# ZhuoyangLiu2005/MLA

Hardware: AMD Instinct MI355X
Metric: training samples/sec + step-time, MLA-Llama2-7B bf16 (higher is better)
Workload: dtype bf16; 1 GPU; BASELINE.json configs[1]: MLA-Llama2-7B SFT, use_pointcloud+use_contrastive, 672x672(+mask) image + 1024 points + 32 text tokens, per-GPU batch 8 x 4 diffusion repeats = 32 x 548 tokens; model=mla-llama2-7b, global_batch=8, seq_len=548, parallelism=single-gpu, activation_save_level=1, optimizer=fused AdamW + grad clip inside the timed region

## Files before the change

include/mla_hip.h:

```cpp
#ifndef MLA_HIP_H
#define MLA_HIP_H

#include <stddef.h>
#include <stdint.h>

#ifdef __cplusplus
extern "C" {
#endif

typedef struct ihipStream_t* mla_stream_t;

const char* mla_last_error(void);
int mla_query(int what);
const char* mla_gemm_source_id(void);
int mla_selftest(const void* src_1k, int* out_tr_256, void* out_glds_1k, mla_stream_t stream);
int mla_calib_mfma(const void* operands, float* out, int blocks, int iters, double* flops_per_launch, mla_stream_t stream);
int mla_dispatch_probe(int* out, int blocks, int hold_us, mla_stream_t stream);

int mla_gemm_bf16(const void* A, const void* B, void* C, const void* R, const void* bias, int M, int N, int K, int lda, int ldb,
                  int ldc, int ldr, int a_mode, int b_mode, int out_fp32, int accumulate, float alpha, int force_generic,
                  mla_stream_t stream);
int mla_gemm_bf16_ws(const void* A, const void* B, void* C, const void* R, const void* bias, int M, int N, int K, int lda, int ldb,
                     int ldc, int ldr, int a_mode, int b_mode, int out_fp32, int accumulate, float alpha, int force_generic,
                     float* workspace, size_t workspace_bytes, mla_stream_t stream);
// ... 32 lines not shown
int mla_colsum_blocks(int rows);
int mla_colsum_bf16(const void* dy, float* out, int accumulate, int rows, int N, int ld, float* workspace, size_t workspace_bytes,
                    mla_stream_t stream);
int mla_layernorm_fwd(const void* x, const void* w, const void* b, void* y, int rows, int H, float eps, mla_stream_t stream);

int mla_rope_inplace(void* buf, const float* cos_t, const float* sin_t, long long tokens, int S, int nheads, int D, int ld,
                     int q_off, int k_off, int backward, mla_stream_t stream);

int mla_swiglu_fwd(const void* gu, void* act, long long rows, int I, mla_stream_t stream);
int mla_swiglu_bwd(const void* dact, const void* gu, void* dgu, void* act_out, long long rows, int I, mla_stream_t stream);
int mla_act_fwd(const void* x, void* y, long long n, int kind, mla_stream_t stream);
int mla_act_bwd(const void* dy, const void* x, void* dx, long long n, int kind, mla_stream_t stream);

int mla_cast_f32_to_bf16(const float* x, void* y, long long n, mla_stream_t stream);
int mla_cast_bf16_to_f32(const void* x, float* y, long long n, mla_stream_t stream);
int mla_add_bf16(const void* a, const void* b, void* y, long long n, mla_stream_t stream);
int mla_gather_rows_bf16(const void* src, const long long* idx, void* out, long long rows, int H, int scatter, mla_stream_t stream);

int mla_transpose_bf16(const void* src, void* dst, long long R, int C, long long ld, long long ldt, mla_stream_t stream);
int mla_rmsnorm_apply_t(const void* x, const void* w, const float* rstd, void* dst, long long rows, int H, long long ldt,
                        mla_stream_t stream);
int mla_swiglu_fwd_t(const void* gu, void* dst, long long rows, int I, long long ldt, mla_stream_t stream);
int mla_swiglu_fwd_dual(const void* gu, void* act, void* actT, long long rows, int I, long long ldt, mla_stream_t stream);
int mla_swiglu_bwd_t(const void* dact, const void* gu, void* dgu, void* dguT, long long rows, int I, long long ldt, mla_stream_t stream);

int mla_embedding_fwd(const long long* ids, const void* table, void* out, long long tokens, int H, int vocab, mla_stream_t stream);
int mla_embedding_bwd(const long long* ids, const void* dy, float* grad, float* workspace, long long tokens, int H, int vocab,
                      mla_stream_t stream);

int mla_adamw_step(float* p, const float* g, float* m, float* v, void* p16, long long n, float lr, float beta1, float beta2,
                   float eps, float weight_decay, int step, const float* grad_scale, mla_stream_t stream);
int mla_adamw_step_groups(float* p, const float* g, float* m, float* v, void* p16, long long n, long long n_decay, float lr, float beta1,
                          float beta2, float eps, float weight_decay, int step, const float* grad_scale, mla_stream_t stream);
int mla_sumsq_f32(const float* x, long long n, float* out, int accumulate, float* workspace, size_t workspace_bytes,
                  mla_stream_t stream);
int mla_sum_partials(const float* partial, int n, float* out, int accumulate, mla_stream_t stream);
int mla_clip_coef(const float* sumsq, float max_norm, float* coef, float* norm_out, mla_stream_t stream);

int mla_q_sample(const float* x0, const float* noise, const long long* t, const float* sqrt_ac, const float* sqrt_1mac, float* out,
                 int batch, int per, int nsteps, mla_stream_t stream);

int mla_attn_fwd(const void* q, const void* k, const void* v, void* o, float* lse, const int* seqlens, int B, int S, int H,
                 int head_dim, long long ld_qkv, long long ld_o, float scale, mla_stream_t stream);
int mla_attn_fwd_g(const void* q, const void* k, const void* v, void* o, float* lse, const int* seqlens, int B, int S, int H,
                   int head_dim, long long ld_qkv, long long ld_o, float scale, int grp_start, int grp_len, const int* grp_starts,
                   mla_stream_t stream);
int mla_attn_bwd_g(const void* q, const void* k, const void* v, const void* o, const void* dout, const float* lse, const int* seqlens,
                   void* dq, void* dk, void* dv, float* delta, int B, int S, int H, int head_dim, long long ld_qkv, long long ld_o,
                   float scale, const float* rope_cos, const float* rope_sin, void* dqT, void* dkT, void* dvT, void* oT,
                   long long ldt, int* head_sync, long long head_sync_ints, int grp_start, int grp_len, const int* grp_starts,
                   int rope_per_sample, mla_stream_t stream);
long long mla_attn_bwd_sync_ints(int B, int H);
int mla_attn_bwd(const void* q, const void* k, const void* v, const void* o, const void* dout, const float* lse, const int* seqlens,
                 void* dq, void* dk, void* dv, float* delta, int B, int S, int H, int head_dim, long long ld_qkv, long long ld_o,
                 float scale, const float* rope_cos, const float* rope_sin, int* head_sync, long long head_sync_ints,
                 mla_stream_t stream);
int mla_attn_bwd_t(const void* q, const void* k, const void* v, const void* o, const void* dout, const float* lse, const int* seqlens,
                   void* dq, void* dk, void* dv, float* delta, int B, int S, int H, int head_dim, long long ld_qkv, long long ld_o,
                   float scale, const float* rope_cos, const float* rope_sin, void* dqT, void* dkT, void* dvT, void* oT,
                   long long ldt, int* head_sync, long long head_sync_ints, mla_stream_t stream);
long long mla_attn_bwd_ws_bytes(int B, int S, int H);
int mla_attn_bwd_ws(const void* q, const void* k, const void* v, const void* o, const void* dout, const float* lse, const int* seqlens,
                    void* dq, void* dk, void* dv, float* delta, int B, int S, int H, int head_dim, long long ld_qkv, long long ld_o,
                    float scale, const float* rope_cos, const float* rope_sin, void* dqT, void* dkT, void* dvT, void* oT, long long ldt,
                    void* ws, long long ws_bytes, mla_stream_t stream);

// ... 93 lines not shown
```

mla_amd/csrc/elementwise.hip:

```cpp
#include "common.h"
#include <math.h>

namespace {


constexpr int NORM_MAXC = 4;

__global__ __launch_bounds__(256) void rmsnorm_fwd_kernel(const bf16_t* __restrict__ x, const bf16_t* __restrict__ w,
                                                          bf16_t* __restrict__ y, float* __restrict__ rstd_out,
                                                          int rows, int H, float eps) {
  __shared__ float scratch[16];
  const int row = blockIdx.x;
  const int nchunk = H >> 3;
  const bf16_t* xr = x + (size_t)row * H;
  float xv[NORM_MAXC][8];
  float ss = 0.f;
#pragma unroll
  for (int c = 0; c < NORM_MAXC; ++c) {
    const int ch = threadIdx.x + c * 256;
    if (ch < nchunk) {
      const u32x4_t v = *(const u32x4_t*)(xr + ch * 8);
      unpack8(v, xv[c]);
#pragma unroll
      for (int j = 0; j < 8; ++j) ss += xv[c][j] * xv[c][j];
// ... 646 lines not shown
          g4[u] = __builtin_nontemporal_load(g + i); p4[u] = __builtin_nontemporal_load(p + i);
          m4[u] = __builtin_nontemporal_load(m + i); v4[u] = __builtin_nontemporal_load(v + i);
        } else {
          g4[u] = g[i]; p4[u] = p[i]; m4[u] = m[i]; v4[u] = v[i];
        }
      }
    }
#pragma unroll
    for (int u = 0; u < UNR; ++u) {
      const long long i = i0 + u * 256;
      if (i >= hi) continue;
      const float decay = i < n4_decay ? decay_on : 1.f;
#pragma unroll
      for (int r = 0; r < 4; ++r) {
        float pp = p4[u][r], mm = m4[u][r], vv = v4[u][r];
        adamw_elem(pp, g4[u][r], mm, vv, gs, decay, beta1, beta2, step, isq, eps);
        p4[u][r] = pp; m4[u][r] = mm; v4[u][r] = vv;
      }
      if (NT) {
        __builtin_nontemporal_store(p4[u], p + i); __builtin_nontemporal_store(m4[u], m + i); __builtin_nontemporal_store(v4[u], v + i);
      } else {
        p[i] = p4[u]; m[i] = m4[u]; v[i] = v4[u];
      }
      if (p16) {
        u32x2_t o;
        o[0] = pack2bf(p4[u][0], p4[u][1]);
        o[1] = pack2bf(p4[u][2], p4[u][3]);
        if (NT) __builtin_nontemporal_store(o, p16 + i); else p16[i] = o;
      }
    }
  }
}

__global__ __launch_bounds__(256) void sumsq_partial_kernel(const float* __restrict__ x, float* __restrict__ partial, long long n) {
  __shared__ float scratch[16];
  float s0 = 0.f, s1 = 0.f;
  const long long n4 = n >> 2;
  const f32x4_t* x4 = (const f32x4_t*)x;
  for (long long i = (long long)blockIdx.x * 256 + threadIdx.x; i < n4; i += (long long)gridDim.x * 256) {
    const f32x4_t v = x4[i];
    s0 += v[0] * v[0] + v[1] * v[1];
    s1 += v[2] * v[2] + v[3] * v[3];
  }
  if (blockIdx.x == 0 && threadIdx.x < (n & 3)) { const float v = x[(n4 << 2) + threadIdx.x]; s0 += v * v; }
  const float s = block_sum(s0 + s1, scratch);
  if (threadIdx.x == 0) partial[blockIdx.x] = s;
}
__global__ __launch_bounds__(256) void sum_final_kernel(const float* __restrict__ partial, float* __restrict__ out, int P,
                                                        int accumulate) {
  __shared__ float scratch[16];
  float s = 0.f;
  int i0 = 0;
  if ((((uintptr_t)partial) & 15) == 0) {
    const f32x4_t* p4 = (const f32x4_t*)partial;
    const int n4 = P >> 2;
    f32x4_t a0 = {0.f, 0.f, 0.f, 0.f}, a1 = a0, a2 = a0, a3 = a0;
    int i = threadIdx.x;
    for (; i + 768 < n4; i += 1024) { a0 += p4[i]; a1 += p4[i + 256]; a2 += p4[i + 512]; a3 += p4[i + 768]; }
    for (; i < n4; i += 256) a0 += p4[i];
    const f32x4_t a = (a0 + a1) + (a2 + a3);
    s = (a[0] + a[1]) + (a[2] + a[3]);
    i0 = n4 << 2;
  }
  for (int i = i0 + threadIdx.x; i < P; i += 256) s += partial[i];
  s = block_sum(s, scratch);
  if (threadIdx.x == 0) out[0] = accumulate ? out[0] + s : s;
// ... 219 lines not shown
  MLA_CHECK_ARG(p && g && m && v && n >= 0 && step >= 1 && n_decay >= 0 && n_decay <= n, "mla_adamw_step: bad args");
  if (n == 0) return 0;
  const float bc1 = 1.f - powf(beta1, (float)step), bc2 = 1.f - powf(beta2, (float)step);
  const long long n4 = (AL16(p) && AL16(g) && AL16(m) && AL16(v) && (p16 == nullptr || ((uintptr_t)p16 & 7) == 0) && (n_decay & 3) == 0) ? n / 4 : 0;
  if (n4) {
    static const int variant = getenv("MLA_ADAMW_VARIANT") ? atoi(getenv("MLA_ADAMW_VARIANT")) : 0;
    const dim3 grid(grid_for(n4, adamw_grid_cap()));
#define ADAMW_LAUNCH(U, N) hipLaunchKernelGGL((adamw_vec4_kernel<U, N>), grid, dim3(256), 0, stream, (f32x4_t*)p, (const f32x4_t*)g, (f32x4_t*)m, \
                       (f32x4_t*)v, (u32x2_t*)p16, n4, lr, beta1, beta2, eps, weight_decay, bc1, bc2, grad_scale, n_decay / 4)
    if (variant == 1) ADAMW_LAUNCH(2, true);
    else if (variant == 9) ADAMW_LAUNCH(1, true);
    else if (variant == 3) ADAMW_LAUNCH(1, false);
    else if (variant == 4) ADAMW_LAUNCH(2, false);
    else ADAMW_LAUNCH(4, true);
#undef ADAMW_LAUNCH
  }
  const long long done = n4 * 4;
  if (done < n)
    hipLaunchKernelGGL(adamw_kernel, dim3(grid_for(n - done, 8192)), dim3(256), 0, stream, p + done, g + done, m + done, v + done,
                       p16 ? (bf16_t*)p16 + done : (bf16_t*)nullptr, n - done, lr, beta1, beta2, eps, weight_decay, bc1, bc2, grad_scale,
                       n_decay > done ? n_decay - done : 0);
  MLA_LAUNCH_CHECK();
}
extern "C" int mla_adamw_step(float* p, const float* g, float* m, float* v, void* p16, long long n, float lr, float beta1,
                              float beta2, float eps, float weight_decay, int step, const float* grad_scale,
                              hipStream_t stream) {
  return adamw_impl(p, g, m, v, p16, n, n, lr, beta1, beta2, eps, weight_decay, step, grad_scale, stream);
}
extern "C" int mla_adamw_step_groups(float* p, const float* g, float* m, float* v, void* p16, long long n, long long n_decay, float lr,
                                     float beta1, float beta2, float eps, float weight_decay, int step, const float* grad_scale,
                                     hipStream_t stream) {
  return adamw_impl(p, g, m, v, p16, n, n_decay, lr, beta1, beta2, eps, weight_decay, step, grad_scale, stream);
}

extern "C" int mla_sumsq_f32(const float* x, long long n, float* out, int accumulate, float* workspace, size_t workspace_bytes,
                             hipStream_t stream) {
  MLA_CHECK_ARG(x && out && workspace && workspace_bytes >= 2048 * sizeof(float) && AL16(x), "mla_sumsq_f32: bad args");
  const int nb = grid_for(n / 4 + 1, 2048);
  hipLaunchKernelGGL(sumsq_partial_kernel, dim3(nb), dim3(256), 0, stream, x, workspace, n);
  hipLaunchKernelGGL(sum_final_kernel, dim3(1), dim3(256), 0, stream, workspace, out, nb, accumulate);
  MLA_LAUNCH_CHECK();
}
extern "C" int mla_sum_partials(const float* partial, int n, float* out, int accumulate, hipStream_t stream) {
  MLA_CHECK_ARG(partial && out && n >= 0, "mla_sum_partials: bad args");
  hipLaunchKernelGGL(sum_final_kernel, dim3(1), dim3(256), 0, stream, partial, out, n, accumulate);
  MLA_LAUNCH_CHECK();
}
extern "C" int mla_clip_coef(const float* sumsq, float max_norm, float* coef, float* norm_out, hipStream_t stream) {
  MLA_CHECK_ARG(sumsq && coef, "mla_clip_coef: bad args");
  hipLaunchKernelGGL(clip_coef_kernel, dim3(1), dim3(1), 0, stream, sumsq, max_norm, coef, norm_out);
  MLA_LAUNCH_CHECK();
}

extern "C" int mla_q_sample(const float* x0, const float* noise, const long long* t, const float* sqrt_ac,
                            const float* sqrt_1mac, float* out, int batch, int per, int nsteps, hipStream_t stream) {
  MLA_CHECK_ARG(x0 && noise && t && sqrt_ac && sqrt_1mac && out, "mla_q_sample: null pointer");
  hipLaunchKernelGGL(q_sample_kernel, dim3((batch * per + 255) / 256), dim3(256), 0, stream, x0, noise, t, sqrt_ac, sqrt_1mac,
                     out, batch, per, nsteps);
  MLA_LAUNCH_CHECK();
}

extern "C" int mla_gather_rows_bf16(const void* src, const long long* idx, void* out, long long rows, int H, int scatter,
                                    hipStream_t stream) {
  MLA_CHECK_ARG(src && idx && out && H % 8 == 0 && AL16(src) && AL16(out), "mla_gather_rows_bf16: bad args");
  hipLaunchKernelGGL(gather_rows_kernel, dim3(grid_for(rows * (H / 8))), dim3(256), 0, stream, (const bf16_t*)src, idx, (bf16_t*)out,
                     rows, H, scatter);
// ... 3 lines not shown
```

mla_amd/fsdp.py:

```python
from __future__ import annotations

from typing import Callable, Dict, List, Optional, Sequence, Tuple

import torch
import torch.distributed as dist
import torch.nn as nn


class HipLocalOps:

    def __init__(self):
        from . import hip
        self.hip = hip

    def cast_to_bf16(self, src32, dst16):
        self.hip.cast_f32_to_bf16(src32, dst16)

    def adamw(self, p32, g32, m, v, p16, lr, betas, eps, wd, step, grad_scale):
        self.hip.adamw_step(p32, g32, m, v, p16, lr, betas[0], betas[1], eps, wd, step, grad_scale)

    def adamw_groups(self, p32, g32, m, v, p16, n_decay, lr, betas, eps, wd, step, grad_scale):
        self.hip.adamw_step_groups(p32, g32, m, v, p16, n_decay, lr, betas[0], betas[1], eps, wd, step, grad_scale)

    def sumsq(self, x32, out1, accumulate):
        self.hip.sumsq(x32, out1, accumulate)

    def sum_partials(self, partials, n, out1, accumulate):
        self.hip.sum_partials(partials, n, out1, accumulate)

    def clip_coef(self, sumsq1, max_norm, coef1, norm1):
        self.hip.clip_coef(sumsq1, max_norm, coef1, norm1)

    def stream(self, device):
        return torch.cuda.Stream(device=device)


class _SqArena:

    def __init__(self, n: int, device):
        self.buf = torch.zeros(n, dtype=torch.float32, device=device)
        self.used = 0

    def take(self, count: int):
        if self.used + count > self.buf.numel():
            return None
        part = self.buf[self.used:self.used + count]
        self.used += count
        return part


def _round_up(n, m):
    return ((n + m - 1) // m) * m


def apply_rccl_env(environ=None) -> Dict[str, str]:
# ... 284 lines not shown
        self.world = dist.get_world_size(process_group) if dist.is_available() and dist.is_initialized() else 1
        self.rank = dist.get_rank(process_group) if self.world > 1 else 0
        self.coll = self.world > 1 or (os.environ.get("MLA_FORCE_COLLECTIVES") == "1" and dist.is_available() and dist.is_initialized())
        self.ops = ops if ops is not None else HipLocalOps()
        if inplace_reduce is None and os.environ.get("MLA_FSDP_INPLACE_RS") == "0":
            inplace_reduce = False
        self.inplace_reduce = bool(self.coll and (dist.get_backend(process_group) == "nccl" if inplace_reduce is None else inplace_reduce))
        self.sum_shards = bool(self.inplace_reduce or (self.coll and dist.get_backend(process_group) == "nccl"))
        self.grad_div = float(self.world) if self.sum_shards else 1.0
        no_decay = no_decay or default_no_decay
        self.units: List[FlatUnit] = []
        self.unit_of_module: Dict[int, FlatUnit] = {}
        found = discover_units(model, unit_policy)
        self._arenas = None
        kinds = [k for k in os.environ.get("MLA_FSDP_ARENAS", "master,exp_avg,exp_avg_sq").split(",") if k and k != "0"]
        if kinds:
            sizes = dict(flat16=0, grad32=0, master=0, exp_avg=0, exp_avg_sq=0, gshard=0)
            for name, mod, named in found:
                _, n_decay, n_train, n_total = plan_flat_layout(named, self.world, no_decay)
                w = self.world if self.coll else 1
                sizes["flat16"] += n_total
                sizes["grad32"] += n_train
                sizes["master"] += n_total // w
                sizes["exp_avg"] += n_train // self.world
                sizes["exp_avg_sq"] += n_train // self.world
                if self.coll and not self.inplace_reduce:
                    sizes["gshard"] += n_train // self.world
            self._arenas = _Arenas({k: v for k, v in sizes.items() if k in kinds}, device, slices=2 * len(found))
        for name, mod, named in found:
            self._add_unit(name, mod, named, no_decay)
        for b in model.buffers():
            b.data = b.data.to(device)
        self.step_count = 0
        self.defer_reduce = False
        self._sumsq = torch.zeros(1, dtype=torch.float32, device=device)
        self._sq_arena = _SqArena(1 << 20, device) if (not self.coll and hasattr(self.ops, "sum_partials") and
                                                       self.device.type == "cuda") else None
        for u in self.units:
            u.sq_arena = self._sq_arena
        self._coef = torch.ones(1, dtype=torch.float32, device=device)
        self._norm = torch.zeros(1, dtype=torch.float32, device=device)
        self.on_gpu = self.device.type == "cuda"
        if self.on_gpu:
            assert torch.cuda.current_device() == (self.device.index or 0), \
                f"torch.cuda.set_device({self.device}) must be called before sharding a model onto it"
        self.comm_stream = self.ops.stream(device) if self.coll else None
        self.wait_profile = None
        if self.on_gpu and self.comm_stream is not None:
            for u in self.units:
                mod = getattr(u, "module", None)
                if mod is not None:
                    mod.register_forward_pre_hook(lambda m, inp, uu=u: self.wait_unit(uu))
                    if hasattr(mod, "_gather_wait"):
                        mod._gather_wait = (lambda uu=u: self.wait_unit(uu))
                else:
                    owned = {id(p) for _, p, _ in u.params}
                    for m in model.modules():
                        if any(id(p) in owned for p in m.parameters(recurse=False)):
                            m.register_forward_pre_hook(lambda mm, inp, uu=u: self.wait_unit(uu))
        for u in self.units:
            mod = getattr(u, "module", None)
            if mod is not None and hasattr(mod, "_grad_hook") and u.trainable and self.coll:
                mod._grad_hook = (lambda uu=u: self._launch_reduce_scatter(uu))

    def _add_unit(self, name, mod, named, no_decay):
        if not named:
# ... 100 lines not shown
                        self._timed_wait("rs_event", u.rs_event)

    def grad_norm_and_clip(self, max_norm: Optional[float]):
        first = True
        small: List[torch.Tensor] = []
        for u in self.units:
            if not u.trainable:
                continue
            if u.sq_entries and not self.coll:
                for a, b in u.uncovered_ranges():
                    if b - a > (1 << 20):
                        self.ops.sumsq(u.gshard[a:b], self._sumsq, not first)
                        first = False
                    else:
                        small.append(u.gshard[a:b])
            else:
                self.ops.sumsq(u.gshard, self._sumsq, not first)
                first = False
        if small:
            self.ops.sumsq(torch.cat(small) if len(small) > 1 else small[0], self._sumsq, not first)
            first = False
        if self._sq_arena is not None and self._sq_arena.used:
            self.ops.sum_partials(self._sq_arena.buf, self._sq_arena.used, self._sumsq, not first)
            first = False
        if self.coll:
            dist.all_reduce(self._sumsq, op=dist.ReduceOp.SUM, group=self.pg)
        if self.grad_div != 1.0:
            self._sumsq.mul_(1.0 / (self.grad_div * self.grad_div))
        self.ops.clip_coef(self._sumsq, float(max_norm) if max_norm is not None else 3.0e38, self._coef, self._norm)
        if self.grad_div != 1.0:
            self._coef.mul_(1.0 / self.grad_div)
        return self._norm

    def optimizer_step(self, lr: float, betas=(0.9, 0.999), eps: float = 1e-8, weight_decay: float = 0.0):
        self.step_count += 1

        for u in self.units:
            if not u.trainable:
                continue
            ranges = u._shard_ranges()
            if hasattr(self.ops, "adamw_groups") and ranges and ranges[0][0] == 0 and \
                    all(ranges[i][1] == ranges[i + 1][0] and ranges[i][2] + (ranges[i][1] - ranges[i][0]) == ranges[i + 1][2]
                        for i in range(len(ranges) - 1)):
                n_local = ranges[-1][1]
                n_dec = sum(le - ls for ls, le, _, dec in ranges if dec)
                g0 = ranges[0][2]
                self.ops.adamw_groups(u.master_train[:n_local], u.gshard[:n_local], u.exp_avg[:n_local], u.exp_avg_sq[:n_local],
                                      u.flat16[g0:g0 + n_local], n_dec, lr, betas, eps, weight_decay, self.step_count, self._coef)
            else:
                for ls, le, g0, decayed in ranges:
                    self.ops.adamw(u.master_train[ls:le], u.gshard[ls:le], u.exp_avg[ls:le], u.exp_avg_sq[ls:le],
                                   u.flat16[g0:g0 + (le - ls)], lr, betas, eps, weight_decay if decayed else 0.0, self.step_count,
                                   self._coef)
            if self.coll:
                if self.on_gpu:
                    ev = torch.cuda.Event()
                    ev.record(torch.cuda.current_stream(self.device))
                    with torch.cuda.stream(self.comm_stream):
                        self.comm_stream.wait_event(ev)
                        self._all_gather(u)
                        u.gather_event = torch.cuda.Event()
                        u.gather_event.record(self.comm_stream)
                else:
                    self._all_gather(u)

    def iter_full_state_fp32(self, to_cpu_on_rank0: bool = False):
        if self.on_gpu:
            self.wait_all()
        for u in self.units:
            full = self._gather_master(u)
            keep = (not to_cpu_on_rank0) or self.rank == 0
            for n, p, o in u.params:
                if not keep:
                    yield n, None
                    continue
                t = full[o:o + p.numel()].view(p.shape)
                yield n, (t.cpu() if to_cpu_on_rank0 else t.clone())
            del full

    def full_state_dict_fp32(self) -> Dict[str, torch.Tensor]:
        return dict(self.iter_full_state_fp32())

    def _gather_master(self, u: FlatUnit):
        if not self.coll:
            return torch.cat([u.master_train, u.master_frozen])
        full = torch.empty(u.n_total, dtype=torch.float32, device=self.device)
        parts_t = [torch.empty(u.shard_train, dtype=torch.float32, device=self.device) for _ in range(self.world)]
        dist.all_gather(parts_t, u.master_train, group=self.pg)
        full[:u.n_train] = torch.cat(parts_t)
        nf = (u.n_total - u.n_train) // self.world
        if nf:
            parts_f = [torch.empty(nf, dtype=torch.float32, device=self.device) for _ in range(self.world)]
            dist.all_gather(parts_f, u.master_frozen, group=self.pg)
            full[u.n_train:] = torch.cat(parts_f)
        return full

    def state_bytes(self):
# ... 2 lines not shown
```

mla_amd/hip.py:

```python
from __future__ import annotations

import ctypes
import os
from ctypes import c_float, c_int, c_longlong, c_size_t, c_void_p
from typing import Optional

import torch

_LIB_PATH = os.environ.get("MLA_HIP_LIB") or os.path.join(os.path.dirname(os.path.abspath(__file__)), "libmla_hip.so")
_lib = None

ACT_GELU_ERF, ACT_GELU_TANH, ACT_RELU, ACT_SILU = 0, 1, 2, 3

SPLITK = os.environ.get("MLA_GEMM_SPLITK", "1") != "0"
SPLITK_WS_BYTES = int(os.environ.get("MLA_GEMM_SPLITK_WS_MB", "64")) << 20

GEMM_PROFILE = None

_SIGNATURES = {
    "mla_query": [c_int],
    "mla_selftest": [c_void_p, c_void_p, c_void_p, c_void_p],
    "mla_dispatch_probe": [c_void_p, c_int, c_int, c_void_p],
    "mla_calib_mfma": [c_void_p, c_void_p, c_int, c_int, c_void_p, c_void_p],
    "mla_gemv_bf16": [c_void_p, c_longlong, c_void_p, c_longlong, c_void_p, c_longlong, c_longlong, c_int, c_void_p, c_longlong, c_int, c_int,
# ... 20 lines not shown
    "mla_gemm_gateup_swiglu": [c_void_p, c_void_p, c_void_p, c_void_p, c_void_p, c_int, c_int, c_int, c_int, c_int, c_longlong,
                               c_void_p],
    "mla_gemm_dact_swiglu_bwd": [c_void_p, c_void_p, c_void_p, c_void_p, c_void_p, c_int, c_int, c_int, c_int, c_int, c_longlong,
                                 c_void_p],
    "mla_rmsnorm_fwd": [c_void_p, c_void_p, c_void_p, c_void_p, c_int, c_int, c_float, c_void_p],
    "mla_rmsnorm_prep": [c_void_p, c_void_p, c_void_p, c_void_p, c_int, c_int, c_float, c_void_p],
    "mla_gemm_res_norm": [c_void_p, c_void_p, c_void_p, c_void_p, c_void_p, c_void_p, c_void_p, c_int, c_int, c_int, c_int, c_int, c_int,
                          c_int, c_void_p, c_size_t, c_void_p],
    "mla_gemm_qkv_rope_rs": [c_void_p, c_void_p, c_void_p, c_int, c_int, c_int, c_int, c_int, c_int, c_void_p, c_void_p, c_int, c_int,
                             c_void_p, c_int, c_float, c_void_p, c_void_p],
    "mla_gemm_gateup_swiglu_rs": [c_void_p, c_void_p, c_void_p, c_void_p, c_void_p, c_int, c_int, c_int, c_int, c_int, c_longlong,
                                  c_void_p, c_int, c_float, c_void_p, c_void_p],
    "mla_rmsnorm_bwd_blocks": [c_int],
    "mla_timm_rmsnorm_fwd": [c_void_p, c_void_p, c_void_p, c_void_p, c_void_p, c_int, c_int, c_float, c_void_p],
    "mla_timm_rmsnorm_bwd": [c_void_p, c_void_p, c_void_p, c_void_p, c_void_p, c_void_p, c_void_p, c_int, c_int, c_int, c_void_p,
                             c_size_t, c_void_p],
    "mla_rmsnorm_bwd": [c_void_p, c_void_p, c_void_p, c_void_p, c_void_p, c_void_p, c_void_p, c_int, c_int, c_int, c_void_p,
                        c_size_t, c_void_p],
    "mla_colsum_blocks": [c_int],
    "mla_colsum_bf16": [c_void_p, c_void_p, c_int, c_int, c_int, c_int, c_void_p, c_size_t, c_void_p],
    "mla_layernorm_fwd": [c_void_p, c_void_p, c_void_p, c_void_p, c_int, c_int, c_float, c_void_p],
    "mla_rope_inplace": [c_void_p, c_void_p, c_void_p, c_longlong, c_int, c_int, c_int, c_int, c_int, c_int, c_int, c_void_p],
    "mla_swiglu_fwd": [c_void_p, c_void_p, c_longlong, c_int, c_void_p],
    "mla_swiglu_bwd": [c_void_p, c_void_p, c_void_p, c_void_p, c_longlong, c_int, c_void_p],
    "mla_act_fwd": [c_void_p, c_void_p, c_longlong, c_int, c_void_p],
    "mla_act_bwd": [c_void_p, c_void_p, c_void_p, c_longlong, c_int, c_void_p],
    "mla_cast_f32_to_bf16": [c_void_p, c_void_p, c_longlong, c_void_p],
    "mla_cast_bf16_to_f32": [c_void_p, c_void_p, c_longlong, c_void_p],
    "mla_add_bf16": [c_void_p, c_void_p, c_void_p, c_longlong, c_void_p],
    "mla_embedding_fwd": [c_void_p, c_void_p, c_void_p, c_longlong, c_int, c_int, c_void_p],
    "mla_embedding_bwd": [c_void_p, c_void_p, c_void_p, c_void_p, c_longlong, c_int, c_int, c_void_p],
    "mla_adamw_step_groups": [c_void_p, c_void_p, c_void_p, c_void_p, c_void_p, c_longlong, c_longlong, c_float, c_float, c_float, c_float,
                              c_float, c_int, c_void_p, c_void_p],
    "mla_adamw_step": [c_void_p, c_void_p, c_void_p, c_void_p, c_void_p, c_longlong, c_float, c_float, c_float, c_float,
                       c_float, c_int, c_void_p, c_void_p],
    "mla_sumsq_f32": [c_void_p, c_longlong, c_void_p, c_int, c_void_p, c_size_t, c_void_p],
    "mla_clip_coef": [c_void_p, c_float, c_void_p, c_void_p, c_void_p],
    "mla_q_sample": [c_void_p, c_void_p, c_void_p, c_void_p, c_void_p, c_void_p, c_int, c_int, c_int, c_void_p],
    "mla_attn_fwd": [c_void_p, c_void_p, c_void_p, c_void_p, c_void_p, c_void_p, c_int, c_int, c_int, c_int, c_longlong,
                     c_longlong, c_float, c_void_p],
    "mla_attn_bwd": [c_void_p, c_void_p, c_void_p, c_void_p, c_void_p, c_void_p, c_void_p, c_void_p, c_void_p, c_void_p,
                     c_void_p, c_int, c_int, c_int, c_int, c_longlong, c_longlong, c_float, c_void_p, c_void_p, c_void_p, c_longlong,
                     c_void_p],
    "mla_attn_bwd_t": [c_void_p, c_void_p, c_void_p, c_void_p, c_void_p, c_void_p, c_void_p, c_void_p, c_void_p, c_void_p,
                       c_void_p, c_int, c_int, c_int, c_int, c_longlong, c_longlong, c_float, c_void_p, c_void_p,
                       c_void_p, c_void_p, c_void_p, c_void_p, c_longlong, c_void_p, c_longlong, c_void_p],
    "mla_attn_bwd_sync_ints": [c_int, c_int],
    "mla_attn_fwd_g": [c_void_p, c_void_p, c_void_p, c_void_p, c_void_p, c_void_p, c_int, c_int, c_int, c_int, c_longlong,
                       c_longlong, c_float, c_int, c_int, c_void_p, c_void_p],
    "mla_attn_bwd_g": [c_void_p, c_void_p, c_void_p, c_void_p, c_void_p, c_void_p, c_void_p, c_void_p, c_void_p, c_void_p,
                       c_void_p, c_int, c_int, c_int, c_int, c_longlong, c_longlong, c_float, c_void_p, c_void_p,
                       c_void_p, c_void_p, c_void_p, c_void_p, c_longlong, c_void_p, c_longlong, c_int, c_int, c_void_p, c_int, c_void_p],
    "mla_attn_bwd_ws_bytes": [c_int, c_int, c_int],
    "mla_attn_bwd_ws": [c_void_p, c_void_p, c_void_p, c_void_p, c_void_p, c_void_p, c_void_p, c_void_p, c_void_p, c_void_p,
                        c_void_p, c_int, c_int, c_int, c_int, c_longlong, c_longlong, c_float, c_void_p, c_void_p,
                        c_void_p, c_void_p, c_void_p, c_void_p, c_longlong, c_void_p, c_longlong, c_void_p],
    "mla_ce_fwd": [c_void_p, c_int, c_longlong, c_void_p, c_void_p, c_void_p, c_int, c_int, c_longlong, c_void_p],
    "mla_ce_bwd": [c_void_p, c_int, c_longlong, c_void_p, c_void_p, c_void_p, c_float, c_void_p, c_longlong, c_int, c_int,
                   c_longlong, c_void_p],
    "mla_infonce_bwd": [c_void_p, c_void_p, c_void_p, c_void_p, c_void_p, c_int, c_int, c_void_p],
    "mla_l2norm_fwd": [c_void_p, c_void_p, c_void_p, c_int, c_int, c_float, c_void_p],
    "mla_l2norm_bwd": [c_void_p, c_void_p, c_void_p, c_void_p, c_int, c_int, c_void_p],
}


def exported_symbols():
# ... 435 lines not shown
    call("mla_cast_bf16_to_f32", _p(x), _p(out), x.numel())
    return out


def add_bf16(a, b):
    y = torch.empty_like(a)
    call("mla_add_bf16", _p(a), _p(b), _p(y), a.numel())
    return y


def embedding_fwd(ids, table):
    tokens = ids.numel()
    vocab, H = table.shape
    out = torch.empty((tokens, H), dtype=torch.bfloat16, device=table.device)
    call("mla_embedding_fwd", _p(ids), _p(table), _p(out), tokens, H, vocab)
    return out


def embedding_bwd(ids, dy2d, grad_f32):
    vocab, H = grad_f32.shape
    tokens = ids.numel()
    ws = torch.empty((tokens // 64, H), dtype=torch.float32, device=grad_f32.device) if tokens >= 64 else None
    call("mla_embedding_bwd", _p(ids), _p(dy2d), _p(grad_f32), _p(ws), tokens, H, vocab)


def adamw_step(p32, g32, m, v, p16, lr, beta1, beta2, eps, wd, step, grad_scale=None):
    call("mla_adamw_step", _p(p32), _p(g32), _p(m), _p(v), _p(p16), p32.numel(), float(lr), float(beta1), float(beta2),
         float(eps), float(wd), int(step), _p(grad_scale))


def adamw_step_groups(p32, g32, m, v, p16, n_decay, lr, beta1, beta2, eps, wd, step, grad_scale=None):
    call("mla_adamw_step_groups", _p(p32), _p(g32), _p(m), _p(v), _p(p16), p32.numel(), int(n_decay), float(lr), float(beta1), float(beta2),
         float(eps), float(wd), int(step), _p(grad_scale))


def sumsq(x32, out1, accumulate):
    ws = workspace(8192, x32.device)
    call("mla_sumsq_f32", _p(x32), x32.numel(), _p(out1), 1 if accumulate else 0, _p(ws), ws.numel())


def clip_coef(sumsq1, max_norm, coef1, norm1=None):
    call("mla_clip_coef", _p(sumsq1), float(max_norm), _p(coef1), _p(norm1))


def q_sample(x0, noise, t, sqrt_ac, sqrt_1mac):
    out = torch.empty_like(x0)
    batch = x0.shape[0]
    call("mla_q_sample", _p(x0), _p(noise), _p(t), _p(sqrt_ac), _p(sqrt_1mac), _p(out), batch, x0.numel() // batch,
         sqrt_ac.numel())
    return out


def _group_args(groups, B):
    start = groups[0]
    if torch.is_tensor(start):
        _req(start, torch.int32, "attention group starts")
        assert start.numel() == B and start.is_contiguous()
        return 0, start
    return int(start), None


def attn_fwd(q, k, v, B, S, H, D, ld_qkv, seqlens, scale, rows=None, groups=None):
    rows = B * S if rows is None else rows
    o = torch.empty((rows, H * D), dtype=torch.bfloat16, device=q.device)
    if rows > B * S:
        o[B * S:].zero_()
# ... 640 lines not shown
```

mla_amd/ops.py:

```python
from __future__ import annotations

import math
import threading
import os
from typing import List, Optional, Sequence

import torch

from . import hip

BF16 = torch.bfloat16


def cat_view(tensors: Sequence[torch.Tensor]) -> Optional[torch.Tensor]:
    if len(tensors) == 1:
        return tensors[0] if tensors[0].is_contiguous() else None
    t0 = tensors[0]
    K = t0.shape[1]
    ptr = t0.data_ptr()
    total = 0
    for t in tensors:
        if t.dim() != 2 or t.shape[1] != K or not t.is_contiguous() or t.data_ptr() != ptr or t.dtype != t0.dtype:
            return None
        if t.untyped_storage().data_ptr() != t0.untyped_storage().data_ptr():
# ... 428 lines not shown

    @staticmethod
    def forward(ctx, a, b, M, temperature):
        _check_bf16_cuda(a, b)
        inv_t = 1.0 / temperature
        L = hip.gemm(a, b, out_dtype=torch.float32, alpha=inv_t)
        Lt = hip.gemm(b, a, out_dtype=torch.float32, alpha=inv_t)
        lr, rl = hip.ce_fwd(L[:M], None, ncols=M)
        lc, cl = hip.ce_fwd(Lt[:M], None, ncols=M)
        ctx.save_for_backward(a, b, L, rl, cl)
        ctx.M, ctx.inv_t = M, inv_t
        return (lr.mean() + lc.mean()) * 0.5

    @staticmethod
    def backward(ctx, g):
        a, b, L, rl, cl = ctx.saved_tensors
        gs = g.to(torch.float32).reshape(1).contiguous()
        dL = hip.infonce_bwd(L, rl, cl, gs, ctx.M)
        da = hip.gemm(dL, b, b_mode=1, alpha=ctx.inv_t) if ctx.needs_input_grad[0] else None
        db = hip.gemm(dL, a, a_mode=1, b_mode=1, alpha=ctx.inv_t) if ctx.needs_input_grad[1] else None
        return da, db, None, None


def info_nce(a, b, M, temperature):
    return InfoNCEFn.apply(a, b, M, temperature)


_ROPE_EPILOGUE = os.environ.get("MLA_ROPE_EPILOGUE", "1") != "0"
_SWIGLU_FWD_EPILOGUE = os.environ.get("MLA_SWIGLU_FWD_EPILOGUE", "1") != "0"
_SWIGLU_BWD_EPILOGUE = os.environ.get("MLA_SWIGLU_BWD_EPILOGUE", "1") != "0"
_ATTN_BWD_T = os.environ.get("MLA_ATTN_BWD_T", "1") != "0"
_SWIGLU_DUAL = os.environ.get("MLA_SWIGLU_DUAL", "1") != "0"
_RECOMPUTE_LEAN = os.environ.get("MLA_RECOMPUTE_LEAN", "1") != "0"


_NORM_FOLD = os.environ.get("MLA_NORM_FOLD", "0") != "0"


def norm_fold_enabled() -> bool:
    return _NORM_FOLD


def set_norm_fold(on: bool) -> bool:
    global _NORM_FOLD
    prev, _NORM_FOLD = _NORM_FOLD, bool(on)
    return prev


class NormFoldIO:
    __slots__ = ("pre", "next_ln", "out")

    def __init__(self, pre=None, next_ln=None):
        self.pre, self.next_ln, self.out = pre, next_ln, None


_ATTN_GROUPS = threading.local()


def current_attn_groups():
    return getattr(_ATTN_GROUPS, "value", None)


class attn_groups:

    def __init__(self, groups):
        self.groups = groups
# ... 140 lines not shown
    def backward(ctx, dout):
        w = ctx.w
        ln1, wq, wk, wv, wo, ln2, wg, wu, wd = w
        B, S, H, nheads, eps = ctx.dims
        seqlens, cos, sin = ctx.aux
        D = H // nheads
        T = B * S
        lvl = ctx.save_level
        xn1 = xn2 = act_ = actT_saved = None
        if lvl >= 2:
            h2, xn1, rstd1, qkv, o, lse, h1, xn2, rstd2, gu, act_ = ctx.saved_tensors
        elif lvl == 1:
            if ctx.has_actT:
                h2, rstd1, qkv, o, lse, h1, rstd2, gu, actT_saved = ctx.saved_tensors
            else:
                h2, rstd1, qkv, o, lse, h1, rstd2, gu = ctx.saved_tensors
        else:
            if ctx.folded:
                h2, rstd1_f = ctx.saved_tensors
            else:
                (h2,), rstd1_f = ctx.saved_tensors, None
            want_t = ctx.needs_input_grad[8 + 8] and _SWIGLU_DUAL and _RECOMPUTE_LEAN
            _, (xn1, rstd1, qkv, o, lse, h1, xn2, rstd2, gu, act_, actT_saved) = DecoderLayerFn._fwd(
                h2, seqlens, cos, sin, B, S, nheads, eps, w, save_t=want_t, groups=ctx.groups, fold=rstd1_f, need_out=not _RECOMPUTE_LEAN)
        need = ctx.needs_input_grad[8:]
        d2 = dout.reshape(T, H)
        if not d2.is_contiguous():
            d2 = d2.contiguous()
        Tr, T = T, _pad_tokens(T)
        if T != Tr:
            d2 = torch.cat([d2, d2.new_zeros(T - Tr, H)], 0)
        grads: List[Optional[torch.Tensor]] = [None] * 9

        def wT(ws):
            wc = cat_view(ws)
            return hip.transpose(wc if wc is not None else torch.cat(list(ws), 0))

        want_w = need[6] or need[7]
        wdT = wT((wd,))
        fused = hip.gemm_dact_swiglu_bwd(d2, wdT, gu) if (want_w and _SWIGLU_BWD_EPILOGUE) else None
        dact = hip.gemm(d2, wdT) if fused is None else None
        del wdT
        if need[8]:
            actT = actT_saved if actT_saved is not None else (hip.swiglu_fwd_t(gu) if act_ is None else hip.transpose(act_))
            grads[8] = deliver_wgrad_nt((wd,), hip.transpose(d2), actT, need[8:9])[0]
            del actT
        act_ = actT_saved = None
        fuse_t = want_w and gu.shape[0] % 8 == 0
        if fused is not None:
            dgu, dguT = fused
        elif fuse_t:
            dgu, dguT = hip.swiglu_bwd_t(dact, gu)
        else:
            dgu, _ = hip.swiglu_bwd(dact, gu)
        del dact, fused
        dxn2 = hip.gemm(dgu, wT((wg, wu)))
        if want_w:
            xn2T = hip.rmsnorm_apply_t(h1, ln2, rstd2) if xn2 is None else hip.transpose(xn2)
            grads[6], grads[7] = deliver_wgrad_nt((wg, wu), dguT if fuse_t else hip.transpose(dgu), xn2T, need[6:8])
            del xn2T
            dguT = None
        del dgu
        xn2 = None
        holder = {}

        def ln2_run(dw_out, acc):
            holder["dh1"] = hip.rmsnorm_bwd(dxn2, h1, ln2, rstd2, dres=d2, dw_out=dw_out, dw_accumulate=acc)

        if need[5]:
# ... 121 lines not shown
            grads[6], grads[7] = deliver_wgrad((wg, wu), dgu_r, xn2_r, need[6:8])
        holder = {}

        def ln2_run(dw_out, acc):
            holder["dh1"] = hip.rmsnorm_bwd(dxn2_r, h1_r, ln2, rstd2_r, dres=d_r, dw_out=dw_out, dw_accumulate=acc)

        if need[5]:
            grads[5] = deliver_vec_grad(ln2, ln2_run)
        else:
            ln2_run(None, False)
        dh1_r = holder["dh1"]
        do_r = hip.gemm(dh1_r, wo, b_mode=1)
        if need[4]:
            grads[4] = deliver_wgrad((wo,), dh1_r, o_r, need[4:5])[0]
        do = hip.gather_rows(do_r[:n], rows, out_rows=T, scatter=True)
        dres = hip.gather_rows(dh1_r[:n], rows, out_rows=T, scatter=True)
        dqkv = torch.empty_like(qkv)
        if T != Tr:
            dqkv[Tr:].zero_()
        fuse_rope = cos.shape[0] in (S, B * S) and cos.is_contiguous() and sin.is_contiguous() and cos.dtype == torch.float32
        want_qkv_w = need[1] or need[2] or need[3]
        tr = None
        if _ATTN_BWD_T and fuse_rope and S % 4 == 0 and want_qkv_w:
            tr = (torch.empty((3 * H, T), dtype=BF16, device=qkv.device), torch.empty((H, T), dtype=BF16, device=qkv.device))
            if T != Tr:
                tr[0][:, Tr:].zero_()
                tr[1][:, Tr:].zero_()
        hip.attn_bwd(qkv[:, :H], qkv[:, H:2 * H], qkv[:, 2 * H:], o, do, lse, seqlens, dqkv[:, :H], dqkv[:, H:2 * H],
                     dqkv[:, 2 * H:], B, S, nheads, D, 3 * H, 1.0 / math.sqrt(D), rope_cos=cos if fuse_rope else None,
                     rope_sin=sin if fuse_rope else None, transposed=tr, groups=ctx.groups)
        del do
        if not fuse_rope:
            hip.rope_inplace(dqkv, cos, sin, cos.shape[0], nheads, D, 0, H, backward=True)
        wqkv = cat_view((wq, wk, wv))
        dxn1 = hip.gemm(dqkv, hip.transpose(wqkv if wqkv is not None else torch.cat([wq, wk, wv], 0)))
        if want_qkv_w:
            xn1T = hip.rmsnorm_apply_t(h2, ln1, rstd1)
            grads[1], grads[2], grads[3] = deliver_wgrad_nt((wq, wk, wv), tr[0] if tr is not None else hip.transpose(dqkv), xn1T, need[1:4])
            del xn1T
        del dqkv, tr

        def ln1_run(dw_out, acc):
            holder["dh"] = hip.rmsnorm_bwd(dxn1, h2, ln1, rstd1, dres=dres, dw_out=dw_out, dw_accumulate=acc)

        if need[0]:
            grads[0] = deliver_vec_grad(ln1, ln1_run)
        else:
            ln1_run(None, False)
        dh = holder["dh"][:Tr].view(B, S, H) if ctx.needs_input_grad[0] else None
        return (dh, None, None, None, None, None, None, *grads)


def decoder_layer_readout(h, seqlens, cos, sin, nheads, eps, rows, weights):
    return ReadoutLayerFn.apply(h, seqlens, cos, sin, nheads, eps, rows, *weights)


def decoder_layer(h, seqlens, cos, sin, nheads, eps, save_level, weights, fold_io=None):
    return DecoderLayerFn.apply(h, seqlens, cos, sin, nheads, eps, save_level, fold_io, *weights)


class GatherRowsFn(torch.autograd.Function):

    @staticmethod
    def forward(ctx, src2d, idx):
        _check_bf16_cuda(src2d)
        ctx.save_for_backward(idx)
        ctx.n_src = src2d.shape[0]
        return hip.gather_rows(src2d.contiguous(), idx)
# ... 438 lines not shown
```

Measured before the change: 14.10 samples/s.

## Emit transposed bf16 weights from AdamW and cache them for backward dgrad

Adds an AdamW kernel that, besides updating fp32 master, moments and the bf16 copy, writes a transposed bf16 copy of each decoder-layer weight matrix through an LDS tile transpose. The backward pass then fetches these cached transposes through a generation-checked lookup, so it no longer runs a transpose kernel per weight in every layer's backward. The cost is extra memory for the transposed copies, an extra write in the optimizer step, and bookkeeping to invalidate the cache when weights are loaded or modified. On steps where the cache is invalid, such as the first, it falls back to transposing.

```diff
diff --git a/include/mla_hip.h b/include/mla_hip.h
--- a/include/mla_hip.h
+++ b/include/mla_hip.h
@@ -88,6 +88,9 @@
                    float eps, float weight_decay, int step, const float* grad_scale, mla_stream_t stream);
 int mla_adamw_step_groups(float* p, const float* g, float* m, float* v, void* p16, long long n, long long n_decay, float lr, float beta1,
                           float beta2, float eps, float weight_decay, int step, const float* grad_scale, mla_stream_t stream);
+int mla_adamw_step_t(float* p, const float* g, float* m, float* v, void* p16, long long n, long long n_decay, const long long* segs,
+                     int nseg, float lr, float beta1, float beta2, float eps, float weight_decay, int step, const float* grad_scale,
+                     mla_stream_t stream);
 int mla_sumsq_f32(const float* x, long long n, float* out, int accumulate, float* workspace, size_t workspace_bytes,
                   mla_stream_t stream);
 int mla_sum_partials(const float* partial, int n, float* out, int accumulate, mla_stream_t stream);
diff --git a/mla_amd/csrc/elementwise.hip b/mla_amd/csrc/elementwise.hip
--- a/mla_amd/csrc/elementwise.hip
+++ b/mla_amd/csrc/elementwise.hip
@@ -702,6 +702,77 @@
   }
 }
 
+struct AdamwTSeg {
+  long long off;
+  long long ldt;
+  bf16_t* wt;
+  int rows, cols;
+  int tile0;
+  int decay;
+};
+constexpr int ADAMW_T_MAXSEG = 8;
+struct AdamwTArgs {
+  AdamwTSeg seg[ADAMW_T_MAXSEG];
+  int nseg;
+};
+
+__global__ __launch_bounds__(256) void adamw_t_kernel(float* __restrict__ p, const float* __restrict__ g, float* __restrict__ m,
+                                                      float* __restrict__ v, bf16_t* __restrict__ p16, AdamwTArgs args, float lr,
+                                                      float beta1, float beta2, float eps, float wd, float bc1, float bc2,
+                                                      const float* __restrict__ grad_scale) {
+  __shared__ unsigned short t[64][66];
+  int s = 0;
+  while (s + 1 < args.nseg && (int)blockIdx.x >= args.seg[s + 1].tile0) ++s;
+  const AdamwTSeg sg = args.seg[s];
+  const int tile = blockIdx.x - sg.tile0, tiles_c = (sg.cols + 63) >> 6;
+  const int r0 = (tile / tiles_c) * 64, c0 = (tile % tiles_c) * 64;
+  const float gs = grad_scale ? *grad_scale : 1.f;
+  const float step = lr / bc1, isq = 1.f / sqrtf(bc2), decay = sg.decay ? 1.f - lr * wd : 1.f;
+  const int tid = threadIdx.x;
+  const int cc = (tid & 15) * 4, rr = tid >> 4;
+  const bool col_ok = c0 + cc < sg.cols;
+  f32x4_t g4[4], p4[4], m4[4], v4[4];
+#pragma unroll
+  for (int it = 0; it < 4; ++it) {
+    const int r = r0 + rr + 16 * it;
+    if (col_ok && r < sg.rows) {
+      const long long i = sg.off + (long long)r * sg.cols + c0 + cc;
+      g4[it] = __builtin_nontemporal_load((const f32x4_t*)(g + i)); p4[it] = __builtin_nontemporal_load((const f32x4_t*)(p + i));
+      m4[it] = __builtin_nontemporal_load((const f32x4_t*)(m + i)); v4[it] = __builtin_nontemporal_load((const f32x4_t*)(v + i));
+    }
+  }
+#pragma unroll
+  for (int it = 0; it < 4; ++it) {
+    const int r = r0 + rr + 16 * it;
+    if (!(col_ok && r < sg.rows)) continue;
+    const long long i = sg.off + (long long)r * sg.cols + c0 + cc;
+#pragma unroll
+    for (int j = 0; j < 4; ++j) {
+      float pp = p4[it][j], mm = m4[it][j], vv = v4[it][j];
+      adamw_elem(pp, g4[it][j], mm, vv, gs, decay, beta1, beta2, step, isq, eps);
+      p4[it][j] = pp; m4[it][j] = mm; v4[it][j] = vv;
+    }
+    __builtin_nontemporal_store(p4[it], (f32x4_t*)(p + i)); __builtin_nontemporal_store(m4[it], (f32x4_t*)(m + i));
+    __builtin_nontemporal_store(v4[it], (f32x4_t*)(v + i));
+    u32x2_t o;
+    o[0] = pack2bf(p4[it][0], p4[it][1]);
+    o[1] = pack2bf(p4[it][2], p4[it][3]);
+    __builtin_nontemporal_store(o, (u32x2_t*)(p16 + i));
+    const int lr_ = rr + 16 * it;
+    t[cc][lr_] = (unsigned short)(o[0] & 0xffffu); t[cc + 1][lr_] = (unsigned short)(o[0] >> 16);
+    t[cc + 2][lr_] = (unsigned short)(o[1] & 0xffffu); t[cc + 3][lr_] = (unsigned short)(o[1] >> 16);
+  }
+  __syncthreads();
+#pragma unroll
+  for (int it = 0; it < 2; ++it) {
+    const int c = (tid >> 3) + it * 32, r = (tid & 7) * 8;
+    if (c0 + c < sg.cols && r0 + r < sg.rows) {
+      const uint32_t* q = (const uint32_t*)&t[c][r];
+      __builtin_nontemporal_store(u32x4_t{q[0], q[1], q[2], q[3]}, (u32x4_t*)(sg.wt + (long long)(c0 + c) * sg.ldt + r0 + r));
+    }
+  }
+}
+
 __global__ __launch_bounds__(256) void sumsq_partial_kernel(const float* __restrict__ x, float* __restrict__ partial, long long n) {
   __shared__ float scratch[16];
   float s0 = 0.f, s1 = 0.f;
@@ -987,6 +1058,49 @@
                                      hipStream_t stream) {
   return adamw_impl(p, g, m, v, p16, n, n_decay, lr, beta1, beta2, eps, weight_decay, step, grad_scale, stream);
 }
+extern "C" int mla_adamw_step_t(float* p, const float* g, float* m, float* v, void* p16, long long n, long long n_decay,
+                                const long long* segs, int nseg, float lr, float beta1, float beta2, float eps, float weight_decay,
+                                int step, const float* grad_scale, hipStream_t stream) {
+  MLA_CHECK_ARG(p && g && m && v && p16 && n >= 0 && step >= 1 && n_decay >= 0 && n_decay <= n, "mla_adamw_step_t: bad args");
+  MLA_CHECK_ARG(segs && nseg >= 1 && nseg <= ADAMW_T_MAXSEG, "mla_adamw_step_t: need 1..%d matrices (got %d)", ADAMW_T_MAXSEG, nseg);
+  MLA_CHECK_ARG(AL16(p) && AL16(g) && AL16(m) && AL16(v) && ((uintptr_t)p16 & 7) == 0, "mla_adamw_step_t: alignment");
+  AdamwTArgs a{};
+  a.nseg = nseg;
+  long long tiles = 0, pos = 0;
+  for (int s = 0; s < nseg; ++s) {
+    const long long off = segs[5 * s], rows = segs[5 * s + 1], cols = segs[5 * s + 2], ldt = segs[5 * s + 4];
+    bf16_t* wt = (bf16_t*)(uintptr_t)segs[5 * s + 3];
+    const long long end = off + rows * cols;
+    MLA_CHECK_ARG(off >= pos && off % 4 == 0 && rows > 0 && cols > 0 && rows % 8 == 0 && cols % 8 == 0 && end <= n &&
+                  rows <= (1 << 30) && cols <= (1 << 30), "mla_adamw_step_t: matrix %d: bad shape or placement", s);
+    MLA_CHECK_ARG(wt && AL16(wt) && ldt % 8 == 0 && ldt >= rows, "mla_adamw_step_t: matrix %d: bad transposed destination", s);
+    MLA_CHECK_ARG(end <= n_decay || off >= n_decay, "mla_adamw_step_t: matrix %d straddles the weight-decay boundary", s);
+    a.seg[s] = AdamwTSeg{off, ldt, wt, (int)rows, (int)cols, (int)tiles, end <= n_decay ? 1 : 0};
+    tiles += ((rows + 63) / 64) * ((cols + 63) / 64);
+    MLA_CHECK_ARG(tiles < (1LL << 31), "mla_adamw_step_t: too many tiles");
+    pos = end;
+  }
+  if (tiles == 0) return 0;
+  const float bc1 = 1.f - powf(beta1, (float)step), bc2 = 1.f - powf(beta2, (float)step);
+  hipLaunchKernelGGL(adamw_t_kernel, dim3((unsigned)tiles), dim3(256), 0, stream, p, g, m, v, (bf16_t*)p16, a, lr, beta1, beta2, eps,
+                     weight_decay, bc1, bc2, grad_scale);
+  {
+    const hipError_t e = hipGetLastError();
+    if (e != hipSuccess) { mla_set_error("mla_adamw_step_t: launch failed: %s", hipGetErrorString(e)); return (int)e; }
+  }
+  pos = 0;
+  for (int s = 0; s <= nseg; ++s) {
+    const long long lo = pos, hi = s < nseg ? a.seg[s].off : n;
+    if (hi > lo) {
+      const long long nd = n_decay <= lo ? 0 : (n_decay >= hi ? hi - lo : n_decay - lo);
+      const int rc = adamw_impl(p + lo, g + lo, m + lo, v + lo, (bf16_t*)p16 + lo, hi - lo, nd, lr, beta1, beta2, eps, weight_decay,
+                                step, grad_scale, stream);
+      if (rc) return rc;
+    }
+    if (s < nseg) pos = a.seg[s].off + (long long)a.seg[s].rows * a.seg[s].cols;
+  }
+  return 0;
+}
 
 extern "C" int mla_sumsq_f32(const float* x, long long n, float* out, int accumulate, float* workspace, size_t workspace_bytes,
                              hipStream_t stream) {
diff --git a/mla_amd/fsdp.py b/mla_amd/fsdp.py
--- a/mla_amd/fsdp.py
+++ b/mla_amd/fsdp.py
@@ -21,6 +21,9 @@
 
     def adamw_groups(self, p32, g32, m, v, p16, n_decay, lr, betas, eps, wd, step, grad_scale):
         self.hip.adamw_step_groups(p32, g32, m, v, p16, n_decay, lr, betas[0], betas[1], eps, wd, step, grad_scale)
+
+    def adamw_t(self, p32, g32, m, v, p16, n_decay, mats, lr, betas, eps, wd, step, grad_scale):
+        self.hip.adamw_step_t(p32, g32, m, v, p16, n_decay, mats, lr, betas[0], betas[1], eps, wd, step, grad_scale)
 
     def sumsq(self, x32, out1, accumulate):
         self.hip.sumsq(x32, out1, accumulate)
@@ -371,6 +374,20 @@
         for b in model.buffers():
             b.data = b.data.to(device)
         self.step_count = 0
+        self.weights_gen = 0
+        self.wt_gen = -1
+        self._wt: Dict[Tuple[int, int, int], torch.Tensor] = {}
+        self._wt_plan: Dict[int, list] = {}
+        import weakref
+        self_ref = weakref.ref(self)
+
+        def loaded(mod, keys):
+            eng = self_ref()
+            if eng is not None:
+                eng.mark_weights_modified()
+        for m in model.modules():
+            if any(True for _ in m.parameters(recurse=False)):
+                m.register_load_state_dict_post_hook(loaded)
         self.defer_reduce = False
         self._sumsq = torch.zeros(1, dtype=torch.float32, device=device)
         self._sq_arena = _SqArena(1 << 20, device) if (not self.coll and hasattr(self.ops, "sum_partials") and
@@ -537,8 +554,49 @@
             self._coef.mul_(1.0 / self.grad_div)
         return self._norm
 
+    def mark_weights_modified(self):
+        self.weights_gen += 1
+
+    def weight_t(self, ws) -> Optional[torch.Tensor]:
+        if self.wt_gen != self.weights_gen:
+            return None
+        return self._wt.get((ws[0].data_ptr(), sum(w.shape[0] for w in ws), ws[0].shape[1]))
+
+    def _wt_mats(self, u: FlatUnit):
+        plan = self._wt_plan.get(id(u))
+        if plan is not None:
+            return plan
+        plan = []
+        mod = getattr(u, "module", None)
+        if mod is not None and hasattr(mod, "self_attn") and hasattr(mod, "mlp"):
+            a, m = mod.self_attn, mod.mlp
+            import weakref
+            for group in ((a.q_proj.weight, a.k_proj.weight, a.v_proj.weight), (a.o_proj.weight,), (m.gate_proj.weight, m.up_proj.weight),
+                          (m.down_proj.weight,)):
+                offs = [u._offset_of.get(id(w)) for w in group]
+                if any(o is None for o in offs) or any(not w.requires_grad or w.dim() != 2 for w in group):
+                    continue
+                rows, cols = [w.shape[0] for w in group], group[0].shape[1]
+                end = offs[-1] + group[-1].numel()
+                if any(w.shape[1] != cols for w in group) or any(offs[i] + group[i].numel() != offs[i + 1] for i in range(len(group) - 1)) \
+                        or end > u.n_train or (offs[0] < u.n_decay < end) or offs[0] % 4 or cols % 8 or any(r % 8 for r in rows):
+                    continue
+                wt = torch.empty((cols, sum(rows)), dtype=torch.bfloat16, device=self.device)
+                self._wt[(group[0].data_ptr(), sum(rows), cols)] = wt
+                group[0]._wt_owner = weakref.ref(self)
+                r0 = 0
+                for w, o, r in zip(group, offs, rows):
+                    plan.append((o, r, cols, wt[:, r0:r0 + r]))
+                    r0 += r
+        self._wt_plan[id(u)] = plan
+        return plan
+
     def optimizer_step(self, lr: float, betas=(0.9, 0.999), eps: float = 1e-8, weight_decay: float = 0.0):
         self.step_count += 1
+        self.weights_gen += 1
+        from . import ops as _ops
+        make_t = _ops._WT_CACHE and not self.coll and self.on_gpu and hasattr(self.ops, "adamw_t")
+        all_t = make_t
 
         for u in self.units:
             if not u.trainable:
@@ -550,9 +608,16 @@
                 n_local = ranges[-1][1]
                 n_dec = sum(le - ls for ls, le, _, dec in ranges if dec)
                 g0 = ranges[0][2]
-                self.ops.adamw_groups(u.master_train[:n_local], u.gshard[:n_local], u.exp_avg[:n_local], u.exp_avg_sq[:n_local],
-                                      u.flat16[g0:g0 + n_local], n_dec, lr, betas, eps, weight_decay, self.step_count, self._coef)
+                mats = self._wt_mats(u) if make_t and g0 == 0 and n_local == u.n_train else None
+                if mats:
+                    self.ops.adamw_t(u.master_train[:n_local], u.gshard[:n_local], u.exp_avg[:n_local], u.exp_avg_sq[:n_local],
+                                     u.flat16[:n_local], n_dec, mats, lr, betas, eps, weight_decay, self.step_count, self._coef)
+                else:
+                    all_t = all_t and not self._wt_plan.get(id(u))
+                    self.ops.adamw_groups(u.master_train[:n_local], u.gshard[:n_local], u.exp_avg[:n_local], u.exp_avg_sq[:n_local],
+                                          u.flat16[g0:g0 + n_local], n_dec, lr, betas, eps, weight_decay, self.step_count, self._coef)
             else:
+                all_t = all_t and not self._wt_plan.get(id(u))
                 for ls, le, g0, decayed in ranges:
                     self.ops.adamw(u.master_train[ls:le], u.gshard[ls:le], u.exp_avg[ls:le], u.exp_avg_sq[ls:le],
                                    u.flat16[g0:g0 + (le - ls)], lr, betas, eps, weight_decay if decayed else 0.0, self.step_count,
@@ -568,6 +633,8 @@
                         u.gather_event.record(self.comm_stream)
                 else:
                     self._all_gather(u)
+        if all_t:
+            self.wt_gen = self.weights_gen
 
     def iter_full_state_fp32(self, to_cpu_on_rank0: bool = False):
         if self.on_gpu:
diff --git a/mla_amd/hip.py b/mla_amd/hip.py
--- a/mla_amd/hip.py
+++ b/mla_amd/hip.py
@@ -76,6 +76,8 @@
     "mla_embedding_bwd": [c_void_p, c_void_p, c_void_p, c_void_p, c_longlong, c_int, c_int, c_void_p],
     "mla_adamw_step_groups": [c_void_p, c_void_p, c_void_p, c_void_p, c_void_p, c_longlong, c_longlong, c_float, c_float, c_float, c_float,
                               c_float, c_int, c_void_p, c_void_p],
+    "mla_adamw_step_t": [c_void_p, c_void_p, c_void_p, c_void_p, c_void_p, c_longlong, c_longlong, c_void_p, c_int, c_float, c_float,
+                         c_float, c_float, c_float, c_int, c_void_p, c_void_p],
     "mla_adamw_step": [c_void_p, c_void_p, c_void_p, c_void_p, c_void_p, c_longlong, c_float, c_float, c_float, c_float,
                        c_float, c_int, c_void_p, c_void_p],
     "mla_sumsq_f32": [c_void_p, c_longlong, c_void_p, c_int, c_void_p, c_size_t, c_void_p],
@@ -577,6 +579,15 @@
 def adamw_step_groups(p32, g32, m, v, p16, n_decay, lr, beta1, beta2, eps, wd, step, grad_scale=None):
     call("mla_adamw_step_groups", _p(p32), _p(g32), _p(m), _p(v), _p(p16), p32.numel(), int(n_decay), float(lr), float(beta1), float(beta2),
          float(eps), float(wd), int(step), _p(grad_scale))
+
+
+def adamw_step_t(p32, g32, m, v, p16, n_decay, mats, lr, beta1, beta2, eps, wd, step, grad_scale=None):
+    segs = (c_longlong * (5 * len(mats)))()
+    for i, (off, rows, cols, wt) in enumerate(mats):
+        assert wt.dtype == torch.bfloat16 and wt.stride(1) == 1 and tuple(wt.shape) == (cols, rows), (tuple(wt.shape), rows, cols)
+        segs[5 * i:5 * i + 5] = [int(off), int(rows), int(cols), wt.data_ptr(), wt.stride(0)]
+    call("mla_adamw_step_t", _p(p32), _p(g32), _p(m), _p(v), _p(p16), p32.numel(), int(n_decay), c_void_p(ctypes.addressof(segs)), len(mats), float(lr), float(beta1),
+         float(beta2), float(eps), float(wd), int(step), _p(grad_scale))
 
 
 def sumsq(x32, out1, accumulate):
diff --git a/mla_amd/ops.py b/mla_amd/ops.py
--- a/mla_amd/ops.py
+++ b/mla_amd/ops.py
@@ -484,6 +484,18 @@
 _ATTN_BWD_T = os.environ.get("MLA_ATTN_BWD_T", "1") != "0"
 _SWIGLU_DUAL = os.environ.get("MLA_SWIGLU_DUAL", "1") != "0"
 _RECOMPUTE_LEAN = os.environ.get("MLA_RECOMPUTE_LEAN", "1") != "0"
+_WT_CACHE = os.environ.get("MLA_WT_CACHE", "1") != "0"
+
+
+def weight_t(ws) -> torch.Tensor:
+    ref = getattr(ws[0], "_wt_owner", None)
+    owner = ref() if ref is not None else None
+    if owner is not None:
+        t = owner.weight_t(ws)
+        if t is not None:
+            return t
+    wc = cat_view(ws)
+    return hip.transpose(wc if wc is not None else torch.cat(list(ws), 0))
 
 
 _NORM_FOLD = os.environ.get("MLA_NORM_FOLD", "0") != "0"
@@ -690,9 +702,7 @@
             d2 = torch.cat([d2, d2.new_zeros(T - Tr, H)], 0)
         grads: List[Optional[torch.Tensor]] = [None] * 9
 
-        def wT(ws):
-            wc = cat_view(ws)
-            return hip.transpose(wc if wc is not None else torch.cat(list(ws), 0))
+        wT = weight_t
 
         want_w = need[6] or need[7]
         wdT = wT((wd,))
@@ -880,8 +890,7 @@
         del do
         if not fuse_rope:
             hip.rope_inplace(dqkv, cos, sin, cos.shape[0], nheads, D, 0, H, backward=True)
-        wqkv = cat_view((wq, wk, wv))
-        dxn1 = hip.gemm(dqkv, hip.transpose(wqkv if wqkv is not None else torch.cat([wq, wk, wv], 0)))
+        dxn1 = hip.gemm(dqkv, weight_t((wq, wk, wv)))
         if want_qkv_w:
             xn1T = hip.rmsnorm_apply_t(h2, ln1, rstd1)
             grads[1], grads[2], grads[3] = deliver_wgrad_nt((wq, wk, wv), tr[0] if tr is not None else hip.transpose(dqkv), xn1T, need[1:4])
```

Result: no change. 14.10 samples/s, median of 5 (-0.0%).
